# haoheliu/AudioLDM2

Measured on AMD Instinct MI355X. Metric: audio_seconds_per_second, higher is better.
Workload: dtype f32 storage/accumulate; each product = 6 bf16 MFMA partial products of exact 3-part operand splits (fp32-grade); 1 GPU; audioldm2-full: batch 8 prompts/GPU x 1 GPU, 10.24 s @16 kHz, 200 DDIM steps, CFG 3.5, eta 1.0, n_candidates 1; one step = sample_log + VAE decode + HiFi-GAN + D2H of the waveform; synthetic conditioning, random-init weights, host-CPU RNG noise; global_batch=8, parallelism=prompt-sharded replicas x1, weight_broadcast_bytes=0

## Files before the change

audioldm2_amd/csrc/api.hip:

```cpp
#include "common.h"
#include <string.h>

namespace aldm {
static thread_local char g_err[512] = "";
void set_error(const char* fmt, ...) {
    va_list ap;
    va_start(ap, fmt);
    vsnprintf(g_err, sizeof(g_err), fmt, ap);
    va_end(ap);
}
}

extern "C" int aldm_version(void) { return 10; }
extern "C" const char* aldm_last_error(void) { return aldm::g_err; }
```

audioldm2_amd/csrc/igemm.hip:

```cpp
#include "igemm_kernel.h"
#include <algorithm>
#include <atomic>
#include <stdlib.h>

namespace aldm {

int igemm_launch_pre0(int BM, int BN, int kgroups, bool uni, bool w8, dim3 grid, hipStream_t st, const IgemmK& p);
int igemm_launch_pre1(int BM, int BN, int kgroups, bool uni, bool w8, dim3 grid, hipStream_t st, const IgemmK& p);
int igemm_launch_pre2(int BM, int BN, int kgroups, bool uni, bool w8, dim3 grid, hipStream_t st, const IgemmK& p);
int igemm_launch_pre3(int BM, int BN, int kgroups, bool uni, bool w8, dim3 grid, hipStream_t st, const IgemmK& p);
int igemm_launch_pre4(int BM, int BN, int kgroups, bool uni, bool w8, dim3 grid, hipStream_t st, const IgemmK& p);
int igemm_launch_bx_pre0(int BM, int BN, int kgroups, bool uni, bool w8, dim3 grid, hipStream_t st, const IgemmK& p);
int igemm_launch_bx_pre1(int BM, int BN, int kgroups, bool uni, bool w8, dim3 grid, hipStream_t st, const IgemmK& p);
int igemm_launch_bx_pre2(int BM, int BN, int kgroups, bool uni, bool w8, dim3 grid, hipStream_t st, const IgemmK& p);
int igemm_launch_bx_pre3(int BM, int BN, int kgroups, bool uni, bool w8, dim3 grid, hipStream_t st, const IgemmK& p);

int igemm_launch_dma(int BM, int BN, int nst, int parts, bool f16, dim3 grid, hipStream_t st, const IgemmK& p);
bool igemm_dma_config_ok(int BM, int BN, int nst, int parts);
#ifdef ALDM_TEST_HOOKS
extern std::atomic<int> g_debug_drop_product;
#endif
int igemm_launch_dma_ws(int BM, int BN, int nst, int parts, int blocks, hipStream_t st, const IgemmK& p);
bool igemm_dma_ws_config_ok(int BM, int BN, int nst, int parts);
int igemm_dma_ws_blocks_per_cu(int BM, int BN, int nst, int parts);
int igemm_launch_dma_lw(int BM, int BN, int nst, int parts, bool f16, dim3 grid, hipStream_t st, const IgemmK& p);
bool igemm_dma_lw_config_ok(int BM, int BN, int nst, int parts);
int igemm_launch_dma_os(int KT, int nst, int parts, bool f16, dim3 grid, hipStream_t st, const IgemmK& p);
bool igemm_dma_os_config_ok(int KT, int nst, int parts);
int igemm_dma_os_default_stages(int KT, int parts);
int igemm_launch_dma_halo(int BM, int BN, int nstb, int wm, int parts, bool f16, int maxch, dim3 grid, hipStream_t st, const IgemmK& p);
int igemm_dma_halo_maxch(int BM, int BN, int nstb, int wm, int parts, int nch);

__global__ __launch_bounds__(256) void igemm_reduce_kernel(const IgemmK p) {
    const aldm_igemm_desc& d = p.d;
    const int z = blockIdx.z;
    const int N4 = d.N >> 2;
// ... 164 lines not shown

static thread_local int g_force_bm = 0, g_force_bn = 0, g_force_splits = 0, g_force_kgroups = 0, g_force_stages = 0;

extern "C" void aldm_igemm_force(int bm, int bn, int splits, int kgroups) {
    g_force_bm = bm;
    g_force_bn = bn;
    g_force_splits = splits;
    g_force_kgroups = kgroups;
    g_force_stages = 0;
}
extern "C" void aldm_igemm_force_stages(int stages) { g_force_stages = stages; }

static int default_wave8_mask() {
    static const int m = [] {
        const char* e = getenv("ALDM_IGEMM_W8");
        return e ? atoi(e) : 1;
    }();
    return m;
}
static thread_local int g_wave8_mask = -1;

extern "C" int aldm_igemm_wave8_mask(int mask) {
    g_wave8_mask = mask;
    return mask < 0 ? default_wave8_mask() : mask;
}

static thread_local int g_force_mma = 0;
extern "C" int aldm_igemm_mma(int mode) {
    const int prev = g_force_mma;
    if (mode >= 0 && mode <= 2) g_force_mma = mode;
    return prev;
}

static int pre_mode_of(const aldm_igemm_desc& d) {
    if (d.pre_scale == nullptr && d.pre_act == ALDM_ACT_NONE) return PRE_NONE;
    if (d.pre_scale != nullptr && d.pre_act == ALDM_ACT_NONE) return PRE_AFFINE;
    if (d.pre_scale != nullptr && d.pre_act == ALDM_ACT_SILU) return PRE_AFFINE_SILU;
    if (d.pre_scale == nullptr && d.pre_act == ALDM_ACT_LRELU) return PRE_LRELU;
    return PRE_GENERIC;
}

static int device_cus() {
    static const int n = [] {
        int dev = 0, cus = 0;
        if (hipGetDevice(&dev) != hipSuccess ||
            hipDeviceGetAttribute(&cus, hipDeviceAttributeMultiprocessorCount, dev) != hipSuccess || cus <= 0)
            return 256;
        return cus;
    }();
    return n;
}

static bool dma_ws_eligible(const IgemmK& p, int BM, int BN) {
    const aldm_igemm_desc& d = p.d;
    const bool geglu = d.epi_mode == ALDM_EPI_GEGLU;
    auto al16 = [](const void* q) { return (reinterpret_cast<uintptr_t>(q) & 15) == 0; };
    if (d.out_mul > 0 || d.accumulate || d.batch != 1 || d.act != ALDM_ACT_NONE || d.out_split_act != ALDM_ACT_NONE ||
        d.epi_mode == ALDM_EPI_QKV)
        return false;
    if (p.M % BM != 0 || d.N % BN != 0 || (d.N & 3) != 0 || (d.ldo & 3) != 0) return false;
    if (!al16(d.out) || !al16(d.res) || !al16(d.bias) || !al16(d.rowbias) || !al16(d.out_split)) return false;
    if (d.rowbias && (p.OHW % BM != 0 || (p.rb_ld & 3) != 0)) return false;
    if (geglu && (BN != 128 || d.res || d.rowbias)) return false;
    return true;
}

static bool dma_os_eligible(const IgemmK& p) {
    const aldm_igemm_desc& d = p.d;
    if (d.KH != 1 || d.KW != 1 || d.SH != 1 || d.SW != 1 || d.PH != 0 || d.PW != 0 || d.up_h != 1 || d.up_w != 1) return false;
    if (d.OH != d.H || d.OW != d.W || d.K != p.Cin || d.K % 32 != 0 || d.out_mul > 0 || d.batch > 1) return false;
    if (d.epi_mode == ALDM_EPI_QKV && d.qkv_c % 128 != 0) return false;
    if (d.rowbias || d.accumulate || d.act != ALDM_ACT_NONE) return false;
    auto al16 = [](const void* q) { return (reinterpret_cast<uintptr_t>(q) & 15) == 0; };
    if ((d.N & 3) != 0 || (d.ldo & 3) != 0 || !al16(d.out) || !al16(d.res)) return false;
    return true;
}

static int dma_halo_chunks(const IgemmK& p, int BM) {
    const aldm_igemm_desc& d = p.d;
    if (d.KH != 3 || d.KW != 3 || d.SH != 1 || d.SW != 1 || d.PH != 1 || d.PW != 1 || d.DH != 1 || d.DW != 1) return 0;
    if (d.up_h != 1 || d.up_w != 1 || d.OH != d.H || d.OW != d.W || d.out_mul > 0 || d.batch > 1) return 0;
    if (d.W <= 0 || (d.W & (d.W - 1)) != 0 || BM % d.W != 0 || p.OHW % BM != 0) return 0;
    return ((BM / d.W + 2) * d.W + 15) / 16;
}

static bool tile_supported(int BM, int BN) {
    return (BM == 128 && (BN == 128 || BN == 64 || BN == 32)) || (BM == 64 && (BN == 128 || BN == 64));
}

static int igemm_prepare(const aldm_igemm_desc* dd, IgemmK& p, int& BM, int& BN) {
    ALDM_CHECK(dd != nullptr, "aldm_igemm: null descriptor");
    p.d = *dd;
    aldm_igemm_desc& d = p.d;
    ALDM_CHECK((d.x1 || d.a_split) && d.w && (d.out || d.out_split), "aldm_igemm: null x1/w/out");
    if (!d.x1) d.x1 = reinterpret_cast<const float*>(d.a_split);
    if (d.split_parts == 0) d.split_parts = 3;
    ALDM_CHECK(d.split_parts == 2 || d.split_parts == 3, "aldm_igemm: split_parts must be 0 / 3 or 2");
    if (d.out_split_parts == 0) d.out_split_parts = d.split_parts;
    ALDM_CHECK(d.out_split_parts == 2 || d.out_split_parts == 3, "aldm_igemm: out_split_parts must be 0, 2 or 3");
    ALDM_CHECK(d.a_fmt == ALDM_FMT_BF16 || (d.a_fmt == ALDM_FMT_F16 && d.a_split != nullptr && d.split_parts == 2 && d.acc_scale > 0.0f),
               "aldm_igemm: a_fmt = ALDM_FMT_F16 needs a pre-split operand (a_split), 2-part images and acc_scale > 0");
    if (d.a_fmt == ALDM_FMT_BF16) d.acc_scale = 1.0f;
    ALDM_CHECK(d.out_split_fmt == ALDM_FMT_BF16 ||
                   (d.out_split_fmt == ALDM_FMT_F16 && d.out_split_scale > 0.0f &&
                    (d.epi_mode == ALDM_EPI_QKV ? (d.k_split != nullptr && d.vt_split != nullptr && d.vt_scale > 0.0f) : d.out_split != nullptr)),
               "aldm_igemm: out_split_fmt = ALDM_FMT_F16 needs out_split (QKV: k_split, vt_split and vt_scale) and out_split_scale > 0");
    if (d.out_split_fmt == ALDM_FMT_F16) d.out_split_parts = 2;
    if (!d.x2) d.C2 = 0;
    if (d.pix1 == 0) d.pix1 = d.C1;
    if (d.pix2 == 0) d.pix2 = d.C2;
    if (d.up_h == 0) d.up_h = 1;
    if (d.up_w == 0) d.up_w = 1;
    if (d.batch == 0) d.batch = 1;
    p.Cin = d.C1 + d.C2;
    ALDM_CHECK(d.C1 > 0 && d.C1 % 4 == 0 && d.C2 % 4 == 0,
               "aldm_igemm: C1=%d/C2=%d must be multiples of 4", d.C1, d.C2);
    ALDM_CHECK(d.pix1 % 4 == 0 && d.pix2 % 4 == 0, "aldm_igemm: pixel pitch must be a multiple of 4");
    ALDM_CHECK(d.K == d.KH * d.KW * p.Cin, "aldm_igemm: K=%d != KH*KW*Cin=%d", d.K,
               d.KH * d.KW * p.Cin);
    ALDM_CHECK(d.N > 0 && (d.ldo >= d.N || d.epi_mode == ALDM_EPI_GEGLU || d.epi_mode == ALDM_EPI_QKV),
               "aldm_igemm: bad N=%d ldo=%d", d.N, d.ldo);
    ALDM_CHECK(d.B > 0 && d.H > 0 && d.W > 0 && d.OH > 0 && d.OW > 0, "aldm_igemm: bad extents");
    ALDM_CHECK(d.SH > 0 && d.SW > 0 && d.DH > 0 && d.DW > 0, "aldm_igemm: bad stride/dilation");
    p.shh = log2_exact(d.up_h);
    p.shw = log2_exact(d.up_w);
// ... 357 lines not shown
    if (splits) *splits = p.splits;
    if (kgroups) *kgroups = p.kgroups;
    if (mma) *mma = p.bx ? ALDM_MMA_BF16X6 : ALDM_MMA_F32;
    return 0;
}

extern "C" int aldm_igemm_plan_stages(const aldm_igemm_desc* dd) {
    IgemmK p;
    int BM, BN;
    if (igemm_prepare(dd, p, BM, BN)) return -1;
    if (p.dma && p.ws == 4) return 400 + (BM == 128 && p.ws_blocks == 4 ? 10 : 0) + p.nst;
    return p.dma ? p.nst + 100 * p.ws : 0;
}

extern "C" int64_t aldm_igemm_ws_floats(const aldm_igemm_desc* dd) {
    if (!dd) return 0;
    aldm_igemm_desc t = *dd;
    t.ws = reinterpret_cast<float*>(uintptr_t(16));
    t.ws_floats = INT64_MAX;
    IgemmK p;
    int BM, BN;
    if (igemm_prepare(&t, p, BM, BN)) return 0;
    return p.splits > 1 ? (int64_t)p.d.batch * p.splits * p.M * p.d.N : 0;
}

extern "C" int aldm_igemm(const aldm_igemm_desc* dd, void* stream) {
    IgemmK p;
    int BM, BN;
    int rc = igemm_prepare(dd, p, BM, BN);
    if (rc) return rc;
    const aldm_igemm_desc& d = p.d;
    dim3 grid((unsigned)(p.tiles_m * p.tiles_n), (unsigned)p.splits, (unsigned)d.batch);
    hipStream_t st = (hipStream_t)stream;
    const int pre = p.pre;
    const bool uni = p.OHW % BM == 0;
    const int env_w8 = g_wave8_mask < 0 ? default_wave8_mask() : g_wave8_mask;
    const bool gn_pre = pre == PRE_AFFINE || pre == PRE_AFFINE_SILU;
    const int tile_bit = (BM == 128 && BN == 128) ? 1 : (BM == 64 && BN == 128) ? 2 : (BM == 128 && BN == 64) ? 4 : 0;
    const bool w8 = p.kgroups == 1 && d.epi_mode != ALDM_EPI_GEGLU && (env_w8 & tile_bit) != 0 &&
                    (p.bx ? tile_bit == 1 : (gn_pre || (tile_bit == 1 && (env_w8 & 8) != 0)));
#ifdef ALDM_TEST_HOOKS
    if (g_debug_drop_product.load(std::memory_order_relaxed))
        ALDM_CHECK(p.dma && p.ws == 0 && BM == 64 && BN == 128 && p.nst == 2 && d.split_parts == 3,
                   "aldm_igemm: aldm_debug_drop_product is set: force the classic DMA-fed 64x128 tile with 2 stages and 3-part images "
                   "(got dma=%d form=%d tile %dx%d, %d stages, %d parts) or clear the switch", p.dma, p.ws, BM, BN, p.nst, d.split_parts);
#endif
    if (p.dma && p.ws == 4) {
        rc = igemm_launch_dma_halo(BM, BN, p.nst, p.ws_blocks, d.split_parts, d.a_fmt == ALDM_FMT_F16, p.os_rows, grid, st, p);
    } else if (p.dma && p.ws == 3) {
        rc = igemm_launch_dma_os(d.K / 32, p.nst, d.split_parts, d.a_fmt == ALDM_FMT_F16, grid, st, p);
    } else if (p.dma && p.ws == 2) {
        rc = igemm_launch_dma_lw(BM, BN, p.nst, d.split_parts, d.a_fmt == ALDM_FMT_F16, grid, st, p);
    } else if (p.dma && p.ws) {
        rc = igemm_launch_dma_ws(BM, BN, p.nst, d.split_parts, p.ws_blocks, st, p);
    } else if (p.dma) {
        rc = igemm_launch_dma(BM, BN, p.nst, d.split_parts, d.a_fmt == ALDM_FMT_F16, grid, st, p);
    } else if (p.bx) {
        switch (pre) {
            case PRE_NONE: rc = igemm_launch_bx_pre0(BM, BN, p.kgroups, uni, w8, grid, st, p); break;
            case PRE_AFFINE: rc = igemm_launch_bx_pre1(BM, BN, p.kgroups, uni, w8, grid, st, p); break;
            case PRE_AFFINE_SILU: rc = igemm_launch_bx_pre2(BM, BN, p.kgroups, uni, w8, grid, st, p); break;
            default: rc = igemm_launch_bx_pre3(BM, BN, p.kgroups, uni, w8, grid, st, p); break;
        }
    } else
    switch (pre) {
        case PRE_NONE: rc = igemm_launch_pre0(BM, BN, p.kgroups, uni, w8, grid, st, p); break;
// ... 102 lines not shown
```

audioldm2_amd/csrc/igemm_dma.h:

```cpp
#pragma once
#include "igemm_epilogue.h"
#include <type_traits>

namespace aldm {

static __device__ __attribute__((aligned(256))) unsigned g_dma_zero_page[256 + 64];

constexpr int dma_stage_slots(int BM, int BN, int NP) { return (BM + BN) * 4 * NP; }
constexpr int dma_lds_bytes(int BM, int BN, int NST, int NP) { return NST * dma_stage_slots(BM, BN, NP) * 16; }
constexpr int dma_blocks_per_cu(int BM, int BN, int NST, int NP) {
    return (160 * 1024) / dma_lds_bytes(BM, BN, NST, NP) >= 2 ? 2 : 1;
}

template <bool F16>
__device__ __forceinline__ f32x16 mfma_32x32x16(const bf16x8 a, const bf16x8 b, const f32x16 c) {
    if constexpr (F16)
        return __builtin_amdgcn_mfma_f32_32x32x16_f16(__builtin_bit_cast(f16x8, a), __builtin_bit_cast(f16x8, b), c, 0, 0, 0);
    else
        return __builtin_amdgcn_mfma_f32_32x32x16_bf16(a, b, c, 0, 0, 0);
}
template <bool F16, int MT, int NT>
__device__ __forceinline__ void unscale_acc(f32x16 (&acc)[MT][NT], float acc_scale) {
    if constexpr (F16) {
#pragma unroll
// ... 281 lines not shown
        if constexpr (ST) issue_dma(st);
        read_frags(f0, st1, 0);
        mma_frags(f1);
#pragma unroll
        for (int q = 0; q < NMF; ++q) {
            __builtin_amdgcn_sched_group_barrier(0x008, 1, 1);
            if (ST && q == 0) __builtin_amdgcn_sched_group_barrier(0x020, D, 1);
            if (q < NRD) __builtin_amdgcn_sched_group_barrier(0x100, 1, 1);
        }
        __builtin_amdgcn_sched_barrier(0);
        if constexpr (ST) advance();
        st = st1;
    };
    for (; t + NST < nk; ++t) body(std::true_type{});
    for (; t + 1 < nk; ++t) body(std::false_type{});
    read_frags(f1, st, 1);
    mma_frags(f0);
    mma_frags(f1);

    __syncthreads();
#if ALDM_DMA_ABLATE & 16
    if (p.M == -12345) {
#pragma unroll
        for (int i = 0; i < MT; ++i)
#pragma unroll
            for (int j = 0; j < NT; ++j)
#pragma unroll
                for (int e = 0; e < 16; ++e) d.ws[(i * NT + j) * 16 + e + threadIdx.x * 256] = acc[i][j][e];
    }
    return;
#endif
    unscale_acc<F16>(acc, d.acc_scale);
    igemm_epilogue<MT, NT>(p, acc, reinterpret_cast<float*>(&smem[0]), m0, n0, wave, wm, wn, lane, 0, split);
}

}
```

audioldm2_amd/csrc/igemm_dma_halo.h:

```cpp
#pragma once
#include "igemm_dma.h"

#ifndef ALDM_HALO_ABLATE
#define ALDM_HALO_ABLATE 0
#endif

namespace aldm {

constexpr int halo_lds_slots(int BN, int NSTB, int NP, int MAXCH) {
    return 2 * MAXCH * NP * 64 + NSTB * BN * 4 * NP + NP * 64;
}

template <int BM, int BN, int NSTB, int WM, int NP, int MAXCH, bool F16 = false>
__global__ __launch_bounds__(128 * WM, WM / 2)
void igemm_dma_halo_kernel(const IgemmK p) {
    constexpr int WN = 2, NW = WM * WN;
    constexpr int MT = BM / (32 * WM), NT = BN / 64;
    constexpr int PB = 64 * NP;
    constexpr int PATCH = MAXCH * NP * 64;
    constexpr int BSTG = BN * 4 * NP;
    constexpr int B0 = 2 * PATCH;
    constexpr int Z0 = B0 + NSTB * BSTG;
    constexpr int NB = 4 * NP * (BN / 64) / NW;
    constexpr int D = NB + 1;
// ... 251 lines not shown
#pragma unroll
        for (int q = 0; q < NMF; ++q) {
            __builtin_amdgcn_sched_group_barrier(0x008, 1, 1);
            if (ST && q == 0) __builtin_amdgcn_sched_group_barrier(0x020, D, 1);
            if (q < NRD) __builtin_amdgcn_sched_group_barrier(0x100, 1, 1);
        }
        __builtin_amdgcn_sched_barrier(0);
        if constexpr (ST) {
            advance_b();
            advance_a();
        }
        st = st1;
    };
    for (; t + NSTB < nk; ++t) body(std::true_type{});
    for (; t + 1 < nk; ++t) body(std::false_type{});
    read_frags(f1, st, 1);
    mma_frags(f0);
    mma_frags(f1);

    __syncthreads();
#if ALDM_DMA_ABLATE & 16
    if (p.M == -12345) {
#pragma unroll
        for (int i = 0; i < MT; ++i)
#pragma unroll
            for (int j = 0; j < NT; ++j)
#pragma unroll
                for (int e = 0; e < 16; ++e) d.ws[(i * NT + j) * 16 + e + threadIdx.x * 256] = acc[i][j][e];
    }
    return;
#endif
    unscale_acc<F16>(acc, d.acc_scale);
    igemm_epilogue<MT, NT>(p, acc, reinterpret_cast<float*>(&smem[0]), m0, n0, wave, wm, wn, lane, 0, split);
}

}
```

audioldm2_amd/csrc/igemm_dma_lw.h:

```cpp
#pragma once
#include "igemm_dma.h"

namespace aldm {

template <int BM, int BN, int NST, int WM, int NP, int BPC, bool F16 = false>
__global__ __launch_bounds__(256 * WM, BPC * WM)
void igemm_dma_lw_kernel(const IgemmK p) {
    constexpr int WN = 2, NW = WM * WN;
    constexpr int MT = BM / (32 * WM), NT = BN / 64;
    constexpr int STG = dma_stage_slots(BM, BN, NP);
    constexpr int PB = 64 * NP;
    constexpr int RA = BM / (16 * NW);
    constexpr int NB = 4 * NP * (BN / 64) / NW;
    constexpr int D = NP * RA + NB;
    constexpr int NPROD = NP == 3 ? 6 : 3;
    static_assert(NP == 2 || NP == 3, "2 or 3 parts");
    static_assert(BM % (16 * NW) == 0 && (4 * NP * (BN / 64)) % NW == 0, "DMA chunks must divide among the loader waves");
    static_assert(NST >= 2 && NST <= 8 && (NST - 1) * D <= 63, "ring depth / vmcnt range");
    static_assert(NW * 32 * (NT * 32 + 4) * 4 <= NST * STG * 16, "epilogue staging must fit the ring");
    __shared__ u32x4 smem[NST * STG];

    const aldm_igemm_desc& d = p.d;
    const int lane = threadIdx.x & 63;
    const int wave_all = __builtin_amdgcn_readfirstlane(threadIdx.x >> 6);
// ... 105 lines not shown
                    t_kw = 0;
                    ++t_kh;
                }
                set_tap();
            }
        };
        auto wait_tiles = [&](int n) {
            constexpr int MX = NST - 1;
            if (n <= 0) wait_vmcnt<0>();
            else if (n == 1) wait_vmcnt<D>();
            else if (n == 2) wait_vmcnt<(MX >= 2 ? 2 : MX) * D>();
            else if (n == 3) wait_vmcnt<(MX >= 3 ? 3 : MX) * D>();
            else if (n == 4) wait_vmcnt<(MX >= 4 ? 4 : MX) * D>();
            else if (n == 5) wait_vmcnt<(MX >= 5 ? 5 : MX) * D>();
            else wait_vmcnt<(MX >= 6 ? 6 : MX) * D>();
        };
#pragma unroll
        for (int s = 0; s < NST; ++s)
            if (s < nk) issue(s);
        wait_tiles(min(nk, NST) - 1);
        __builtin_amdgcn_s_barrier();
        int st = 0, t = 0;
        for (; t + NST < nk; ++t) {
            wait_vmcnt<(NST - 2) * D>();
            __builtin_amdgcn_s_barrier();
            issue(st);
            st = st + 1 == NST ? 0 : st + 1;
        }
        for (; t + 1 < nk; ++t) {
            wait_tiles(min(NST - 2, nk - 2 - t));
            __builtin_amdgcn_s_barrier();
        }
        __builtin_amdgcn_s_barrier();
        return;
    }

    struct Frag {
        bf16x8 a[MT][NP], b[NT][NP];
    };
    const int a_sw = (l31 >> 2) & 3;
    auto read_frags = [&](Frag& f, int st, int step) {
        const u32x4* sa = &smem[st * STG];
        const int o = 2 * step + lh;
#pragma unroll
        for (int i = 0; i < MT; ++i) {
            const int row = (wm * MT + i) * 32 + l31;
#pragma unroll
            for (int q = 0; q < NP; ++q)
                f.a[i][q] = __builtin_bit_cast(bf16x8, sa[((row >> 4) * NP + q) * 64 + (row & 15) * 4 + (o ^ a_sw)]);
        }
#pragma unroll
        for (int j = 0; j < NT; ++j)
#pragma unroll
            for (int q = 0; q < NP; ++q)
                f.b[j][q] = __builtin_bit_cast(bf16x8, sa[BM * 4 * NP + (o * NP + q) * BN + (wn * NT + j) * 32 + l31]);
    };
    f32x16 acc[MT][NT];
#pragma unroll
    for (int i = 0; i < MT; ++i)
#pragma unroll
        for (int j = 0; j < NT; ++j)
#pragma unroll
            for (int e = 0; e < 16; ++e) acc[i][j][e] = 0.f;
    auto mma_frags = [&](const Frag& f) {
        constexpr int PA_[6] = {NP == 3 ? 0 : 1, NP == 3 ? 2 : 0, NP == 3 ? 1 : 0, 0, 1, 0};
        constexpr int PB_[6] = {NP == 3 ? 2 : 0, NP == 3 ? 0 : 1, NP == 3 ? 1 : 0, 1, 0, 0};
// ... 46 lines not shown
```

audioldm2_amd/csrc/igemm_dma_os.h:

```cpp
#pragma once
#include "igemm_dma.h"

#ifndef ALDM_OS_ABLATE
#define ALDM_OS_ABLATE 0
#endif

#ifndef ALDM_OS_GEGLU_PACK
#define ALDM_OS_GEGLU_PACK 1
#endif

namespace aldm {

constexpr int os_stage_slots(int KT, int NP) { return KT * 128 * NP; }
constexpr int OS_EPI_SLOTS = 512;
constexpr int os_lds_bytes(int KT, int NST, int NP) { return (NST * os_stage_slots(KT, NP) + OS_EPI_SLOTS) * 16; }

enum { OS_EPI_PLAIN = 0, OS_EPI_GEGLU = 1, OS_EPI_QKV = 2 };

template <int KT, int NST, int NP, int EPI, int NPO = NP, bool F16 = false, bool FO = false>
__global__ __launch_bounds__(512, 2)
void igemm_dma_os_kernel(const IgemmK p) {
    constexpr int STG = os_stage_slots(KT, NP);
    constexpr int PB = 64 * NP;
    constexpr int NPROD = NP == 3 ? 6 : 3;
// ... 256 lines not shown
#pragma unroll
                for (int rt = 0; rt < 2; ++rt)
#pragma unroll
                    for (int q = 0; q < NP; ++q)
                        af[kn & 1][rt][q] = __builtin_bit_cast(bf16x8, sa[kn * 128 * NP + (rt * NP + q) * 64 + foff]);
                __builtin_amdgcn_sched_barrier(0);
            }
            if (!(ALDM_OS_ABLATE & 2)) {
#pragma unroll
                for (int q = 1; q < NPROD; ++q)
#pragma unroll
                    for (int rt = 0; rt < 2; ++rt)
                        acc[rt] = mfma16(af[kt & 1][rt][PA_[q]], bw[kt][PB_[q]], acc[rt]);
            } else {
#pragma unroll
                for (int rt = 0; rt < 2; ++rt)
#pragma unroll
                    for (int q = 0; q < NP; ++q) asm volatile("" ::"v"(af[kt & 1][rt][q]), "v"(bw[kt][q]));
            }
            __builtin_amdgcn_sched_barrier(0);
        }
        if constexpr (F16) {
            acc[0] *= d.acc_scale;
            acc[1] *= d.acc_scale;
        }
        if (t + 1 < nstg) {
            if (more) wait_vmcnt<(NST - 2) * ND>();
            else wait_vmcnt<0>();
        }
        if (!late) epilogue(t);
        __builtin_amdgcn_s_barrier();
    }
    if (late) epilogue(nstg - 1);
}

}
```

audioldm2_amd/csrc/igemm_epilogue.h:

```cpp
#pragma once
#include "common.h"

#ifndef ALDM_DMA_ABLATE
#define ALDM_DMA_ABLATE 0
#endif

namespace aldm {

struct IgemmK {
    aldm_igemm_desc d;
    int Cin, M, OHW, HV, WV, shh, shw, Kg, Npad, tiles_m, tiles_n;
    int splits, kt_per_split;
    int kgroups;
    int rb_ld;
    int bx;
    int pre;
    int dma;
    int nst;
    int ws;
    int ws_blocks;
    int os_rows;
};

enum { PRE_NONE = 0, PRE_AFFINE = 1, PRE_AFFINE_SILU = 2, PRE_LRELU = 3, PRE_GENERIC = 4 };

using bf16x8 = __bf16 __attribute__((ext_vector_type(8)));
using u32x2 = unsigned __attribute__((ext_vector_type(2)));
using u32x4 = unsigned __attribute__((ext_vector_type(4)));
__device__ __forceinline__ unsigned hi16_pair(unsigned a, unsigned b) { return __builtin_amdgcn_perm(b, a, 0x07060302u); }

constexpr int SPLIT_BLOCK_BYTES = 192;

__device__ __forceinline__ unsigned bf16_rn_bits(float x) {
    const unsigned u = __builtin_bit_cast(unsigned, x);
    return (u + 0x7FFFu + ((u >> 16) & 1u)) & 0xFFFF0000u;
}

__device__ __forceinline__ void split4(const f32x4 v, u32x2 (&part)[3]) {
    unsigned u0[4], u1[4], u2[4];
#pragma unroll
    for (int c = 0; c < 4; ++c) {
        const float x = v[c];
        u0[c] = __builtin_bit_cast(unsigned, x);
        const float r1 = x - __builtin_bit_cast(float, u0[c] & 0xFFFF0000u);
        u1[c] = __builtin_bit_cast(unsigned, r1);
        const float r2 = r1 - __builtin_bit_cast(float, u1[c] & 0xFFFF0000u);
        u2[c] = __builtin_bit_cast(unsigned, r2);
    }
    part[0] = u32x2{hi16_pair(u0[0], u0[1]), hi16_pair(u0[2], u0[3])};
    part[1] = u32x2{hi16_pair(u1[0], u1[1]), hi16_pair(u1[2], u1[3])};
    part[2] = u32x2{hi16_pair(u2[0], u2[1]), hi16_pair(u2[2], u2[3])};
}

using bf16x4 = __bf16 __attribute__((ext_vector_type(4)));
__device__ __forceinline__ void split4_rn2(const f32x4 v, u32x2 (&part)[3]) {
// ... 325 lines not shown
```

audioldm2_amd/ddim.py:

```python
from __future__ import annotations

import gc
import os

import numpy as np
import torch

from . import ops


def make_ddim_timesteps(ddim_discr_method, num_ddim_timesteps, num_ddpm_timesteps, verbose=True):
    if ddim_discr_method == "uniform":
        c = num_ddpm_timesteps // num_ddim_timesteps
        ddim_timesteps = np.asarray(list(range(0, num_ddpm_timesteps, c)))
    elif ddim_discr_method == "quad":
        ddim_timesteps = ((np.linspace(0, np.sqrt(num_ddpm_timesteps * 0.8), num_ddim_timesteps)) ** 2).astype(int)
    else:
        raise NotImplementedError(f'There is no ddim discretization method called "{ddim_discr_method}"')
    return ddim_timesteps + 1


def make_ddim_sampling_parameters(alphacums, ddim_timesteps, eta, verbose=True):
    alphas = alphacums[ddim_timesteps]
    alphas_prev = np.asarray([alphacums[0]] + alphacums[ddim_timesteps[:-1]].tolist())
    sigmas = eta * np.sqrt((1 - alphas_prev) / (1 - alphas) * (1 - alphas / alphas_prev))
    return torch.as_tensor(np.asarray(sigmas, dtype=np.float64)), alphas, alphas_prev


class GraphStepper:

    def __init__(self, fn, use_graph=True):
        self.fn, self.use_graph, self.calls, self.graph = fn, use_graph, 0, None

    def __call__(self):
        if self.use_graph and self.calls >= 1:
            if self.graph is None:
                g = torch.cuda.CUDAGraph()
                torch.cuda.synchronize()
                gc.collect()
                gc_was_on = gc.isenabled()
                gc.disable()
                try:
                    with torch.cuda.graph(g, capture_error_mode="thread_local"):
                        self.fn()
                    self.graph = g
                except RuntimeError as e:
                    import sys
                    print(f"[audioldm2_amd] HIP graph capture failed ({e}); continuing without a graph",
                          file=sys.stderr, flush=True)
                    self.use_graph = False
                    torch.cuda.synchronize()
                    if gc_was_on:
                        gc.enable()
                    self.fn()
                    self.calls += 1
                    return
                finally:
                    if gc_was_on:
                        gc.enable()
            self.graph.replay()
        else:
            self.fn()
        self.calls += 1


def drop_graph_entries(cache: dict) -> None:
    for ent in list(cache.values()):
        rs = ent.get("run_step")
        if rs is not None:
            rs.fn = None
            rs.graph = None
        ent.clear()
    cache.clear()


class _NoiseFeed:

    def __init__(self, draw, steps, shape, with_mask, temperature, dev, chunk=8, mask_first=True, noise_buf=None,
                 qnoise_buf=None, threaded=None):
        import threading
        self.draw, self.steps, self.with_mask, self.temperature = draw, steps, with_mask, temperature
        self.mask_first = mask_first
        self.bounds = [0, min(1, steps)]
        while self.bounds[-1] < steps:
            self.bounds.append(min(steps, self.bounds[-1] + chunk))
        self.chunk = chunk
        self.noise = noise_buf if noise_buf is not None else torch.empty((steps,) + tuple(shape), device=dev,
                                                                         dtype=torch.float32)
        assert self.noise.shape == (steps,) + tuple(shape)
        self.qnoise = (qnoise_buf if qnoise_buf is not None else torch.empty_like(self.noise)) if with_mask else None
        nbuf = 3
        self.pin = [torch.empty((chunk,) + tuple(shape)).pin_memory() for _ in range(nbuf)]
        self.qpin = [torch.empty((chunk,) + tuple(shape)).pin_memory() for _ in range(nbuf)] if with_mask else None
        self.stream = torch.cuda.Stream(device=dev)
        self.stream.wait_stream(torch.cuda.current_stream())
        self.noise.record_stream(self.stream)
        if self.qnoise is not None:
            self.qnoise.record_stream(self.stream)
        self.events = {}
# ... 232 lines not shown
            drop_graph_entries(unet._graph_cache)
            ent = None
        if ent is not None:
            for dst, src in zip(ent["prepared"]["ctxs"] + ent["prepared"]["masks"],
                                prepared["ctxs"] + prepared["masks"]):
                dst.copy_(src)
            if prepared["y"] is not None:
                ent["prepared"]["y"].copy_(prepared["y"])
            unet.refresh_context_kv(ent["kv"])
            ent["x_cur"].copy_(img)
            ent["coef_all"].copy_(coef)
            ent["t_tab"].copy_(t_tab)
        else:
            ent = {"x_cur": img.clone(), "pred_x0": torch.empty_like(img), "t_cur": t_tab[0].clone(),
                   "step_idx": torch.zeros(1, device=dev, dtype=torch.int32), "coef_all": coef.clone(), "t_tab": t_tab.clone(),
                   "noise_all": torch.empty((total_steps,) + tuple(shape), device=dev, dtype=torch.float32),
                   "prepared": prepared}

            def step(e=ent):
                x_c = e["x_cur"]
                if use_cfg:
                    if cfg_fused:
                        eps = self.model.apply_model_cfg(x_c, e["t_cur"], cond, unconditional_conditioning,
                                                         prepared=e["prepared"])
                    else:
                        tl = e["t_cur"][:b].long()
                        e_u = self.model.apply_model(x_c, tl, unconditional_conditioning)
                        e_c = self.model.apply_model(x_c, tl, cond)
                        eps = torch.stack([e_u, e_c]).contiguous()
                else:
                    eps = self.model.apply_model(x_c, e["t_cur"][:b].long(), cond).contiguous()
                ops.ddim_step_indexed(x_c, eps, e["noise_all"], e["coef_all"], e["step_idx"], e["pred_x0"])
                ops.step_advance(e["step_idx"], e["t_tab"], e["t_cur"])
            ent["run_step"] = GraphStepper(step, self.use_graph)
            if can_cache:
                drop_graph_entries(unet._graph_cache)
                unet._graph_cache[key] = ent
        ent["step_idx"].zero_()
        ent["t_cur"].copy_(ent["t_tab"][0])
        x_cur, pred_x0 = ent["x_cur"], ent["pred_x0"]
        cb_rng = any(getattr(f, "uses_rng", True) for f in (callback, img_callback) if f is not None)
        feed = _NoiseFeed(draw, total_steps, tuple(shape), mask is not None, temperature, dev, noise_buf=ent["noise_all"],
                          **({"threaded": False, "chunk": 1} if cb_rng else {}))
        feed.produce_next()
        qn = feed.qnoise
        run_step = ent["run_step"]
        intermediates = {"x_inter": [img], "pred_x0": [img]}
        try:
            for i, step_t in enumerate(time_range):
                index = total_steps - i - 1
                opens_chunk = feed.wait(i)
                if mask is not None:
                    ops.inpaint_blend(x_cur, x0_d, qn[i], mask_d, blend_coef[i])
                run_step()
                if can_cache and ent.get("kv") is None:
                    ent["kv"] = unet.collect_context_kv(ent["prepared"]["ctxs"])
                if opens_chunk and not cb_rng:
                    feed.produce_next()
                if callback:
                    callback(i)
                if img_callback:
                    img_callback(pred_x0, i)
                if index % log_every_t == 0 or index == total_steps - 1:
                    intermediates["x_inter"].append(x_cur.clone())
                    intermediates["pred_x0"].append(pred_x0.clone())
        finally:
            feed.close()
# ... 63 lines not shown
```

audioldm2_amd/lib.py:

```python
from __future__ import annotations

import ctypes as C
import os

_HERE = os.path.dirname(os.path.abspath(__file__))
LIB_PATH = os.environ.get("ALDM_LIB_PATH") or os.path.join(_HERE, "libaldm_hip.so")
ABI_VERSION = 10

ACT_NONE, ACT_SILU, ACT_LRELU, ACT_TANH, ACT_LOGCLAMP, ACT_GELU, ACT_GELU_TANH = range(7)
B_PACKED, B_NT = 0, 1
EPI_PLAIN, EPI_GEGLU, EPI_QKV = 0, 1, 2
FMT_BF16, FMT_F16 = 0, 1


class IgemmDesc(C.Structure):

    _fields_ = [
        ("x1", C.c_void_p), ("x2", C.c_void_p),
        ("C1", C.c_int32), ("C2", C.c_int32),
        ("pix1", C.c_int32), ("pix2", C.c_int32),
        ("B", C.c_int32), ("H", C.c_int32), ("W", C.c_int32),
        ("up_h", C.c_int32), ("up_w", C.c_int32),
        ("KH", C.c_int32), ("KW", C.c_int32), ("SH", C.c_int32), ("SW", C.c_int32),
        ("PH", C.c_int32), ("PW", C.c_int32), ("DH", C.c_int32), ("DW", C.c_int32),
        ("OH", C.c_int32), ("OW", C.c_int32),
        ("pre_scale", C.c_void_p), ("pre_shift", C.c_void_p),
        ("pre_act", C.c_int32), ("pre_slope", C.c_float),
        ("w", C.c_void_p),
        ("b_mode", C.c_int32), ("ldb", C.c_int32),
        ("K", C.c_int32), ("N", C.c_int32),
        ("bias", C.c_void_p), ("rowbias", C.c_void_p), ("res", C.c_void_p), ("out", C.c_void_p),
        ("ldo", C.c_int32), ("act", C.c_int32), ("act_slope", C.c_float), ("alpha", C.c_float),
        ("accumulate", C.c_int32),
        ("out_mul", C.c_int32), ("out_off", C.c_int32), ("out_len", C.c_int32),
        ("batch", C.c_int32),
        ("stride_x", C.c_int64), ("stride_w", C.c_int64), ("stride_o", C.c_int64),
        ("rowbias_ld", C.c_int32), ("epi_mode", C.c_int32),
        ("ws", C.c_void_p), ("ws_floats", C.c_int64),
        ("hint_bm", C.c_int32), ("hint_bn", C.c_int32), ("hint_splits", C.c_int32), ("hint_kgroups", C.c_int32),
        ("w_split", C.c_void_p), ("hint_mma", C.c_int32), ("hint_stages", C.c_int32),
        ("a_split", C.c_void_p), ("out_split", C.c_void_p), ("out_split_c", C.c_int32), ("split_parts", C.c_int32),
        ("out_split_act", C.c_int32), ("out_split_slope", C.c_float),
        ("k_split", C.c_void_p), ("vt_split", C.c_void_p), ("qkv_c", C.c_int32), ("qkv_rows", C.c_int32),
        ("a_fmt", C.c_int32), ("acc_scale", C.c_float), ("out_split_parts", C.c_int32),
        ("out_split_fmt", C.c_int32), ("out_split_scale", C.c_float), ("vt_scale", C.c_float),
    ]


_SIGS = {
    "aldm_version": (C.c_int, []),
    "aldm_last_error": (C.c_char_p, []),
    "aldm_igemm": (C.c_int, [C.POINTER(IgemmDesc), C.c_void_p]),
    "aldm_igemm_plan": (C.c_int, [C.POINTER(IgemmDesc), C.POINTER(C.c_int), C.POINTER(C.c_int),
                                  C.POINTER(C.c_int64), C.POINTER(C.c_int), C.POINTER(C.c_int),
                                  C.POINTER(C.c_int)]),
    "aldm_igemm_ws_floats": (C.c_int64, [C.POINTER(IgemmDesc)]),
    "aldm_igemm_plan_stages": (C.c_int, [C.POINTER(IgemmDesc)]),
    "aldm_igemm_force": (None, [C.c_int, C.c_int, C.c_int, C.c_int]),
    "aldm_igemm_force_stages": (None, [C.c_int]),
    "aldm_igemm_wave8_mask": (C.c_int, [C.c_int]),
    "aldm_split_image_bytes": (C.c_int64, [C.c_int64, C.c_int, C.c_int]),
    "aldm_split_rows": (C.c_int, [C.c_void_p, C.c_void_p, C.c_int, C.c_int, C.c_int64, C.c_int, C.c_void_p, C.c_void_p,
                                  C.c_int, C.c_void_p, C.c_void_p, C.c_int, C.c_void_p]),
    "aldm_split_rows_act": (C.c_int, [C.c_void_p, C.c_void_p, C.c_int, C.c_int, C.c_int64, C.c_int, C.c_void_p, C.c_void_p,
                                      C.c_int, C.c_float, C.c_void_p, C.c_void_p, C.c_int, C.c_void_p]),
    "aldm_layernorm_split": (C.c_int, [C.c_void_p, C.c_void_p, C.c_void_p, C.c_int, C.c_int, C.c_void_p, C.c_void_p,
                                       C.c_float, C.c_int, C.c_void_p]),
    "aldm_attention_d32_split": (C.c_int, [C.c_void_p, C.c_void_p, C.c_void_p, C.c_void_p, C.c_void_p, C.c_int, C.c_int,
                                           C.c_int, C.c_int, C.c_int, C.c_int, C.c_int, C.c_int, C.c_int,
                                           C.c_void_p, C.c_float, C.c_void_p]),
    "aldm_split_bytes_parts": (C.c_int64, [C.c_int, C.c_int, C.c_int]),
    "aldm_pack_split_bf16_parts": (C.c_int, [C.c_void_p, C.c_void_p, C.c_int, C.c_int, C.c_int, C.c_void_p]),
    "aldm_pack_split_f16": (C.c_int, [C.c_void_p, C.c_void_p, C.c_int, C.c_int, C.c_float, C.c_void_p]),
    "aldm_split_rows_f16": (C.c_int, [C.c_void_p, C.c_void_p, C.c_int, C.c_int, C.c_int64, C.c_int, C.c_void_p, C.c_void_p,
                                      C.c_int, C.c_float, C.c_void_p, C.c_void_p, C.c_int, C.c_float, C.c_void_p]),
    "aldm_groupnorm_split_f16": (C.c_int, [C.c_void_p, C.c_void_p, C.c_int, C.c_int, C.c_int, C.c_int, C.c_int, C.c_float,
                                           C.c_void_p, C.c_void_p, C.c_int, C.c_void_p, C.c_void_p, C.c_void_p, C.c_void_p,
                                           C.c_void_p, C.c_int, C.c_float, C.c_void_p]),
    "aldm_layernorm_split_f16": (C.c_int, [C.c_void_p, C.c_void_p, C.c_void_p, C.c_int, C.c_int, C.c_void_p, C.c_void_p,
                                           C.c_float, C.c_float, C.c_void_p]),
    "aldm_igemm_mma": (C.c_int, [C.c_int]),
    "aldm_split_bytes": (C.c_int64, [C.c_int, C.c_int]),
    "aldm_pack_split_bf16": (C.c_int, [C.c_void_p, C.c_void_p, C.c_int, C.c_int, C.c_void_p]),
    "aldm_pack_weight": (C.c_int, [C.c_void_p, C.c_void_p, C.c_int, C.c_int, C.c_int, C.c_int,
                                   C.c_int, C.c_int, C.c_int, C.c_void_p]),
    "aldm_pack_kn": (C.c_int, [C.c_void_p, C.c_void_p, C.c_int, C.c_int, C.c_int, C.c_int,
                               C.c_int64, C.c_int64, C.c_void_p]),
    "aldm_groupnorm_stats": (C.c_int, [C.c_void_p, C.c_void_p, C.c_int, C.c_int, C.c_int, C.c_int,
                                       C.c_int, C.c_float, C.c_void_p, C.c_void_p, C.c_void_p,
                                       C.c_void_p, C.c_void_p, C.c_void_p]),
    "aldm_gn_ws_floats": (C.c_int64, [C.c_int, C.c_int, C.c_int, C.c_int]),
    "aldm_groupnorm_split": (C.c_int, [C.c_void_p, C.c_void_p, C.c_int, C.c_int, C.c_int, C.c_int, C.c_int, C.c_float,
                                       C.c_void_p, C.c_void_p, C.c_int, C.c_void_p, C.c_void_p, C.c_void_p, C.c_void_p,
# ... 136 lines not shown
```

include/aldm_hip.h:

```cpp
#ifndef ALDM_HIP_H
#define ALDM_HIP_H

#include <stdint.h>

#ifdef __cplusplus
extern "C" {
#endif

int aldm_version(void);
const char* aldm_last_error(void);

enum {
    ALDM_ACT_NONE = 0,
    ALDM_ACT_SILU = 1,
    ALDM_ACT_LRELU = 2,
    ALDM_ACT_TANH = 3,
    ALDM_ACT_LOGCLAMP = 4,
    ALDM_ACT_GELU = 5,
    ALDM_ACT_GELU_TANH = 6
};

enum { ALDM_EPI_PLAIN = 0, ALDM_EPI_GEGLU = 1, ALDM_EPI_QKV = 2 };

enum {
// ... 39 lines not shown
    int32_t hint_bm, hint_bn, hint_splits;
    int32_t hint_kgroups;
    const void* w_split;
    int32_t hint_mma;
    int32_t hint_stages;
    const void* a_split;
    void* out_split;
    int32_t out_split_c;
    int32_t split_parts;
    int32_t out_split_act;
    float out_split_slope;
    void* k_split;
    void* vt_split;
    int32_t qkv_c;
    int32_t qkv_rows;
    int32_t a_fmt;
    float acc_scale;
    int32_t out_split_parts;
    int32_t out_split_fmt;
    float out_split_scale;
    float vt_scale;
} aldm_igemm_desc;

int aldm_igemm(const aldm_igemm_desc* d, void* stream);
int64_t aldm_igemm_ws_floats(const aldm_igemm_desc* d);
enum { ALDM_FMT_BF16 = 0, ALDM_FMT_F16 = 1 };
int aldm_igemm_plan(const aldm_igemm_desc* d, int* bm, int* bn, int64_t* flops, int* splits, int* kgroups,
                    int* mma);
int aldm_igemm_plan_stages(const aldm_igemm_desc* d);
void aldm_igemm_force(int bm, int bn, int splits, int kgroups);
void aldm_igemm_force_stages(int stages);
int aldm_igemm_wave8_mask(int mask);
int aldm_igemm_mma(int mode);
#ifdef ALDM_TEST_HOOKS
int aldm_debug_drop_product(int on);
#endif
int64_t aldm_split_bytes(int K, int N);
int aldm_pack_split_bf16(const float* packed, void* dst, int K, int N, void* stream);
int64_t aldm_split_bytes_parts(int K, int N, int parts);
int aldm_pack_split_bf16_parts(const float* packed, void* dst, int K, int N, int parts, void* stream);
int aldm_pack_split_f16(const float* packed, void* dst, int K, int N, float scale, void* stream);

int64_t aldm_split_image_bytes(int64_t rows, int C, int parts);
int aldm_split_rows(const float* x1, const float* x2, int C1, int C2, int64_t rows, int P, const float* scale,
                    const float* shift, int act, void* dst, void* dst_raw, int parts, void* stream);
int aldm_split_rows_act(const float* x1, const float* x2, int C1, int C2, int64_t rows, int P, const float* scale,
                        const float* shift, int act, float slope, void* dst, void* dst_raw, int parts, void* stream);
int aldm_split_rows_f16(const float* x1, const float* x2, int C1, int C2, int64_t rows, int P, const float* scale,
                        const float* shift, int act, float slope, void* dst, void* dst_raw, int raw_parts, float f16_scale,
                        void* stream);

int aldm_pack_weight(const float* src, float* dst, int N, int Cin, int KH, int KW,
                     int transposed, int phase, int stride, void* stream);
int aldm_pack_kn(const float* src, float* dst, int K, int N, int lds, int batch,
                 int64_t stride_src, int64_t stride_dst, void* stream);

int aldm_groupnorm_stats(const float* x1, const float* x2, int B, int P, int C1, int C2,
                         int G, float eps, const float* gamma, const float* beta,
                         float* scale, float* shift, float* ws, void* stream);
int64_t aldm_gn_ws_floats(int B, int P, int C, int G);
int aldm_groupnorm_split(const float* x1, const float* x2, int B, int P, int C1, int C2, int G, float eps,
                         const float* gamma, const float* beta, int act, float* scale, float* shift, float* ws,
                         void* dst, void* dst_raw, int parts, void* stream);
int aldm_groupnorm_split_f16(const float* x1, const float* x2, int B, int P, int C1, int C2, int G, float eps,
                             const float* gamma, const float* beta, int act, float* scale, float* shift, float* ws,
                             void* dst, void* dst_raw, int raw_parts, float f16_scale, void* stream);
// ... 84 lines not shown
```

Baseline: 18.84 audio-s/s.

## Prefetch next GEMM's weights into cache from tail of current igemm kernel

Records the sequence of split-weight pointers used by igemm during the first DDIM step, then during graph capture replays that plan so each igemm kernel, after its epilogue, issues dummy global loads over the next GEMM's weight image. This warms L2/MALL so the following kernel's weight reads hit cache instead of HBM. It adds tail work and extra memory traffic to every kernel, depends on the call order staying identical, and the footprint can be capped through environment variables.

```diff
diff --git a/audioldm2_amd/csrc/api.hip b/audioldm2_amd/csrc/api.hip
--- a/audioldm2_amd/csrc/api.hip
+++ b/audioldm2_amd/csrc/api.hip
@@ -11,5 +11,5 @@
 }
 }
 
-extern "C" int aldm_version(void) { return 10; }
+extern "C" int aldm_version(void) { return 11; }
 extern "C" const char* aldm_last_error(void) { return aldm::g_err; }
diff --git a/audioldm2_amd/csrc/igemm.hip b/audioldm2_amd/csrc/igemm.hip
--- a/audioldm2_amd/csrc/igemm.hip
+++ b/audioldm2_amd/csrc/igemm.hip
@@ -2,6 +2,7 @@
 #include <algorithm>
 #include <atomic>
 #include <stdlib.h>
+#include <vector>
 
 namespace aldm {
 
@@ -232,6 +233,77 @@
     return prev;
 }
 
+struct WplanEntry {
+    const char* w;
+    int64_t bytes;
+    int64_t tile_bytes;
+};
+enum { WPLAN_OFF = 0, WPLAN_RECORD = 1, WPLAN_PLAY = 2, WPLAN_LOST = 3 };
+static thread_local std::vector<WplanEntry> g_wplan;
+static thread_local int g_wplan_mode = WPLAN_OFF, g_wplan_pos = 0, g_wplan_lead = 1, g_wplan_played = 0, g_wplan_mismatched = 0;
+
+static void wplan_cap(int64_t& cap_bytes, int& cap_tiles) {
+    static const int64_t kb = [] {
+        const char* e = getenv("ALDM_WPREFETCH_CAP_KB");
+        return e ? atoll(e) : 0ll;
+    }();
+    static const int tiles = [] {
+        const char* e = getenv("ALDM_WPREFETCH_CAP_TILES");
+        return e ? atoi(e) : 4;
+    }();
+    cap_bytes = kb * 1024;
+    cap_tiles = tiles > 0 ? tiles : 1;
+}
+
+extern "C" void aldm_wplan_record(void) {
+    g_wplan.clear();
+    g_wplan_mode = WPLAN_RECORD;
+    g_wplan_pos = g_wplan_played = g_wplan_mismatched = 0;
+}
+extern "C" void aldm_wplan_play(int lead) {
+    g_wplan_mode = WPLAN_PLAY;
+    g_wplan_lead = lead > 0 ? lead : 1;
+    g_wplan_pos = g_wplan_played = g_wplan_mismatched = 0;
+}
+extern "C" void aldm_wplan_stop(int* played, int* mismatched) {
+    if (played) *played = g_wplan_played;
+    if (mismatched) *mismatched = g_wplan_mismatched;
+    g_wplan_mode = WPLAN_OFF;
+}
+
+static void wplan_step(IgemmK& p) {
+    const aldm_igemm_desc& d = p.d;
+    const char* w = reinterpret_cast<const char*>(d.w_split);
+    if (g_wplan_mode == WPLAN_RECORD) {
+        g_wplan.push_back({w, aldm_split_bytes_parts(d.K, d.N, d.split_parts), (int64_t)4 * d.split_parts * p.Npad * 16});
+        return;
+    }
+    if (g_wplan_mode == WPLAN_LOST) {
+        ++g_wplan_mismatched;
+        return;
+    }
+    if (g_wplan_mode != WPLAN_PLAY) return;
+    const size_t n = g_wplan.size();
+    if ((size_t)g_wplan_pos >= n || g_wplan[g_wplan_pos].w != w) {
+        g_wplan_mode = WPLAN_LOST;
+        ++g_wplan_mismatched;
+        return;
+    }
+    const WplanEntry& e = g_wplan[((size_t)g_wplan_pos + g_wplan_lead) % n];
+    int64_t cap_bytes, bytes = e.bytes;
+    int cap_tiles;
+    wplan_cap(cap_bytes, cap_tiles);
+    if (cap_bytes > 0 && bytes > cap_bytes) bytes = std::min(bytes, cap_tiles * e.tile_bytes);
+    const uintptr_t lo = (reinterpret_cast<uintptr_t>(e.w) + 127) & ~(uintptr_t)127;
+    const uintptr_t hi = (reinterpret_cast<uintptr_t>(e.w) + (uintptr_t)bytes) & ~(uintptr_t)127;
+    if (hi > lo && hi - lo < ((uintptr_t)1 << 37)) {
+        p.pf_ptr = reinterpret_cast<const char*>(lo);
+        p.pf_bytes = (int64_t)(hi - lo);
+    }
+    ++g_wplan_played;
+    ++g_wplan_pos;
+}
+
 static int pre_mode_of(const aldm_igemm_desc& d) {
     if (d.pre_scale == nullptr && d.pre_act == ALDM_ACT_NONE) return PRE_NONE;
     if (d.pre_scale != nullptr && d.pre_act == ALDM_ACT_NONE) return PRE_AFFINE;
@@ -291,6 +363,8 @@
 static int igemm_prepare(const aldm_igemm_desc* dd, IgemmK& p, int& BM, int& BN) {
     ALDM_CHECK(dd != nullptr, "aldm_igemm: null descriptor");
     p.d = *dd;
+    p.pf_ptr = nullptr;
+    p.pf_bytes = 0;
     aldm_igemm_desc& d = p.d;
     ALDM_CHECK((d.x1 || d.a_split) && d.w && (d.out || d.out_split), "aldm_igemm: null x1/w/out");
     if (!d.x1) d.x1 = reinterpret_cast<const float*>(d.a_split);
@@ -714,6 +788,7 @@
     const aldm_igemm_desc& d = p.d;
     dim3 grid((unsigned)(p.tiles_m * p.tiles_n), (unsigned)p.splits, (unsigned)d.batch);
     hipStream_t st = (hipStream_t)stream;
+    if (d.a_split) wplan_step(p);
     const int pre = p.pre;
     const bool uni = p.OHW % BM == 0;
     const int env_w8 = g_wave8_mask < 0 ? default_wave8_mask() : g_wave8_mask;
diff --git a/audioldm2_amd/csrc/igemm_dma.h b/audioldm2_amd/csrc/igemm_dma.h
--- a/audioldm2_amd/csrc/igemm_dma.h
+++ b/audioldm2_amd/csrc/igemm_dma.h
@@ -337,6 +337,7 @@
 #endif
     unscale_acc<F16>(acc, d.acc_scale);
     igemm_epilogue<MT, NT>(p, acc, reinterpret_cast<float*>(&smem[0]), m0, n0, wave, wm, wn, lane, 0, split);
-}
-
-}
+    wprefetch_touch(p, threadIdx.x, NW * 64);
+}
+
+}
diff --git a/audioldm2_amd/csrc/igemm_dma_halo.h b/audioldm2_amd/csrc/igemm_dma_halo.h
--- a/audioldm2_amd/csrc/igemm_dma_halo.h
+++ b/audioldm2_amd/csrc/igemm_dma_halo.h
@@ -307,6 +307,7 @@
 #endif
     unscale_acc<F16>(acc, d.acc_scale);
     igemm_epilogue<MT, NT>(p, acc, reinterpret_cast<float*>(&smem[0]), m0, n0, wave, wm, wn, lane, 0, split);
+    wprefetch_touch(p, threadIdx.x, NW * 64);
 }
 
 }
diff --git a/audioldm2_amd/csrc/igemm_dma_lw.h b/audioldm2_amd/csrc/igemm_dma_lw.h
--- a/audioldm2_amd/csrc/igemm_dma_lw.h
+++ b/audioldm2_amd/csrc/igemm_dma_lw.h
@@ -161,6 +161,7 @@
             __builtin_amdgcn_s_barrier();
         }
         __builtin_amdgcn_s_barrier();
+        wprefetch_touch(p, wave * 64 + lane, NW * 64);
         return;
     }
 
diff --git a/audioldm2_amd/csrc/igemm_dma_os.h b/audioldm2_amd/csrc/igemm_dma_os.h
--- a/audioldm2_amd/csrc/igemm_dma_os.h
+++ b/audioldm2_amd/csrc/igemm_dma_os.h
@@ -312,6 +312,7 @@
         __builtin_amdgcn_s_barrier();
     }
     if (late) epilogue(nstg - 1);
+    else wprefetch_touch(p, threadIdx.x, 256);
 }
 
 }
diff --git a/audioldm2_amd/csrc/igemm_epilogue.h b/audioldm2_amd/csrc/igemm_epilogue.h
--- a/audioldm2_amd/csrc/igemm_epilogue.h
+++ b/audioldm2_amd/csrc/igemm_epilogue.h
@@ -20,7 +20,23 @@
     int ws;
     int ws_blocks;
     int os_rows;
+    const char* pf_ptr;
+    int64_t pf_bytes;
 };
+
+__device__ __forceinline__ void wprefetch_touch(const IgemmK& p, int tid, int nthr) {
+    const int nlines = (int)(p.pf_bytes >> 7);
+    if (nlines == 0) return;
+    const int G = gridDim.x * gridDim.y;
+    const int b = blockIdx.y * gridDim.x + blockIdx.x;
+    const int64_t step = (int64_t)G * nthr;
+    unsigned sink = 0;
+    for (int64_t i = b + (int64_t)G * tid; i < nlines; i += step) {
+        const char* q = p.pf_ptr + (i << 7);
+        asm volatile("global_load_dword %0, %1, off" : "+v"(sink) : "v"(q) : "memory");
+    }
+    asm volatile("" ::"v"(sink));
+}
 
 enum { PRE_NONE = 0, PRE_AFFINE = 1, PRE_AFFINE_SILU = 2, PRE_LRELU = 3, PRE_GENERIC = 4 };
 
diff --git a/audioldm2_amd/ddim.py b/audioldm2_amd/ddim.py
--- a/audioldm2_amd/ddim.py
+++ b/audioldm2_amd/ddim.py
@@ -27,12 +27,52 @@
     return torch.as_tensor(np.asarray(sigmas, dtype=np.float64)), alphas, alphas_prev
 
 
+_wplan_owner = None
+WPLAN_LEAD = 1
+
+
+def wplan_enabled() -> bool:
+    return os.environ.get("ALDM_WPREFETCH", "1") != "0"
+
+
+def wplan_drop() -> None:
+    global _wplan_owner
+    _wplan_owner = None
+    from . import lib
+    if lib._lib is not None:
+        lib._lib.aldm_wplan_record()
+        lib._lib.aldm_wplan_stop(None, None)
+
+
 class GraphStepper:
 
-    def __init__(self, fn, use_graph=True):
+    def __init__(self, fn, use_graph=True, wplan=False):
         self.fn, self.use_graph, self.calls, self.graph = fn, use_graph, 0, None
+        self.wplan = wplan and wplan_enabled()
+        self.wplan_counts = None
 
     def __call__(self):
+        if not self.wplan or (self.calls >= 1 and self.use_graph and self.graph is not None):
+            return self._call()
+        global _wplan_owner
+        from . import lib
+        l = lib.load()
+        if self.calls == 0:
+            l.aldm_wplan_record()
+            _wplan_owner = self
+        elif _wplan_owner is self:
+            l.aldm_wplan_play(int(os.environ.get("ALDM_WPREFETCH_LEAD", WPLAN_LEAD)))
+        else:
+            return self._call()
+        try:
+            self._call()
+        finally:
+            import ctypes
+            played, missed = ctypes.c_int(0), ctypes.c_int(0)
+            l.aldm_wplan_stop(ctypes.byref(played), ctypes.byref(missed))
+            self.wplan_counts = (played.value, missed.value)
+
+    def _call(self):
         if self.use_graph and self.calls >= 1:
             if self.graph is None:
                 g = torch.cuda.CUDAGraph()
@@ -65,6 +105,7 @@
 
 
 def drop_graph_entries(cache: dict) -> None:
+    wplan_drop()
     for ent in list(cache.values()):
         rs = ent.get("run_step")
         if rs is not None:
@@ -363,7 +404,7 @@
                     eps = self.model.apply_model(x_c, e["t_cur"][:b].long(), cond).contiguous()
                 ops.ddim_step_indexed(x_c, eps, e["noise_all"], e["coef_all"], e["step_idx"], e["pred_x0"])
                 ops.step_advance(e["step_idx"], e["t_tab"], e["t_cur"])
-            ent["run_step"] = GraphStepper(step, self.use_graph)
+            ent["run_step"] = GraphStepper(step, self.use_graph, wplan=True)
             if can_cache:
                 drop_graph_entries(unet._graph_cache)
                 unet._graph_cache[key] = ent
diff --git a/audioldm2_amd/lib.py b/audioldm2_amd/lib.py
--- a/audioldm2_amd/lib.py
+++ b/audioldm2_amd/lib.py
@@ -5,7 +5,7 @@
 
 _HERE = os.path.dirname(os.path.abspath(__file__))
 LIB_PATH = os.environ.get("ALDM_LIB_PATH") or os.path.join(_HERE, "libaldm_hip.so")
-ABI_VERSION = 10
+ABI_VERSION = 11
 
 ACT_NONE, ACT_SILU, ACT_LRELU, ACT_TANH, ACT_LOGCLAMP, ACT_GELU, ACT_GELU_TANH = range(7)
 B_PACKED, B_NT = 0, 1
@@ -59,6 +59,9 @@
     "aldm_igemm_force": (None, [C.c_int, C.c_int, C.c_int, C.c_int]),
     "aldm_igemm_force_stages": (None, [C.c_int]),
     "aldm_igemm_wave8_mask": (C.c_int, [C.c_int]),
+    "aldm_wplan_record": (None, []),
+    "aldm_wplan_play": (None, [C.c_int]),
+    "aldm_wplan_stop": (None, [C.POINTER(C.c_int), C.POINTER(C.c_int)]),
     "aldm_split_image_bytes": (C.c_int64, [C.c_int64, C.c_int, C.c_int]),
     "aldm_split_rows": (C.c_int, [C.c_void_p, C.c_void_p, C.c_int, C.c_int, C.c_int64, C.c_int, C.c_void_p, C.c_void_p,
                                   C.c_int, C.c_void_p, C.c_void_p, C.c_int, C.c_void_p]),
diff --git a/include/aldm_hip.h b/include/aldm_hip.h
--- a/include/aldm_hip.h
+++ b/include/aldm_hip.h
@@ -95,6 +95,9 @@
 void aldm_igemm_force_stages(int stages);
 int aldm_igemm_wave8_mask(int mask);
 int aldm_igemm_mma(int mode);
+void aldm_wplan_record(void);
+void aldm_wplan_play(int lead);
+void aldm_wplan_stop(int* played, int* mismatched);
 #ifdef ALDM_TEST_HOOKS
 int aldm_debug_drop_product(int on);
 #endif
```

Measured after the change: 18.88 audio-s/s (median of 4 runs). Within noise of the previous version (+0.2%).
